# cxzheng/sprsolve

Measured on AMD Instinct MI355X. Metric: BiCGStab iterations/s (f64, 50M-row 7-point 3-D Poisson) + CSR SpMV GB/s vs HBM roofline, higher is better.
Workload: dtype f64

## Files before the change

### sprsolve_amd/csrc/capi.hip

```cpp
#include <sys/mman.h>

#include <cstdlib>
#include <memory>
#include <new>
#include <string>

#include "krylov.hpp"

using namespace sprs;

static_assert(sizeof(sprs_c64) == sizeof(cplx), "Complex<f64> layout");
static_assert(sizeof(sprs_c32) == sizeof(cplxf), "Complex<f32> layout");

#define SPRS_GUARD_BEGIN try {
#define SPRS_GUARD_END                         \
    }                                          \
    catch (const std::bad_alloc &) {           \
        return SPRS_ERR_HIP;                   \
    }                                          \
    catch (...) {                              \
        return SPRS_ERR_HIP;                   \
    }

extern "C" {
// ... 53 lines not shown
    (void)hipSetDevice(c->device);
    (void)hipStreamSynchronize(c->stream);
    if (c->d_part) (void)hipFree(c->d_part);
    if (c->d_scal) (void)hipFree(c->d_scal);
    if (c->h_scal) (void)hipHostFree(c->h_scal);
    if (c->own_stream && c->stream) (void)hipStreamDestroy(c->stream);
    delete c;
    return SPRS_OK;
}

int sprs_ctx_sync(sprs_ctx *c) {
    if (!c) return SPRS_INVALID_ARGUMENT;
    SPRS_HIP_TRY(c, hipStreamSynchronize(c->stream));
    return SPRS_OK;
}

const char *sprs_last_error(const sprs_ctx *c) { return c ? c->err : "null context"; }

int sprs_ctx_set(sprs_ctx *c, const char *key, int64_t value) {
    if (!c || !key) return SPRS_INVALID_ARGUMENT;
    std::string k(key);
    if (k == "grid") { if (value < 8 || value > MAX_GRID) return SPRS_INVALID_ARGUMENT; c->grid = (int)(value & ~7); }
    else if (k == "spmv_grid") { if (value > MAX_GRID / 2 || (value >= 0 && value < 8)) return SPRS_INVALID_ARGUMENT; c->spmv_grid = value < 0 ? -1 : (int)(value & ~7); }
    else if (k == "xcd_chunk") c->xcd_chunk = value < 0 ? -1 : (value ? 1 : 0);
    else if (k == "spmv_dict") { if (value < -1 || value > 2) return SPRS_INVALID_ARGUMENT; c->spmv_dict = (int)value; }
    else if (k == "spmv_wide") c->spmv_wide = value < 0 ? -1 : (value ? 1 : 0);
    else if (k == "spmv_uniform") c->spmv_uniform = value < 0 ? -1 : (value ? 1 : 0);
    else if (k == "spmv_period") c->spmv_period = value < 0 ? -1 : (value ? 1 : 0);
    else if (k == "spmv_triple") c->spmv_triple = value < 0 ? -1 : (value ? 1 : 0);
    else if (k == "spmv_seam") c->spmv_seam = value < 0 ? -1 : (value ? 1 : 0);
    else if (k == "spmv_tile") c->spmv_tile = value < 0 ? -1 : (value ? 1 : 0);
    else if (k == "spmv_chain") c->spmv_chain = value < 0 ? -1 : (value ? 1 : 0);
    else if (k == "spmv_fuse") c->spmv_fuse = value < 0 ? -1 : (value ? 1 : 0);
    else if (k == "bicg_k5") { if (value > 2) return SPRS_INVALID_ARGUMENT; c->bicg_k5 = value < 0 ? -1 : (int)value; }
    else if (k == "p2p_allreduce") c->p2p_allreduce = value < 0 ? -1 : (value ? 1 : 0);
    else if (k == "p2p_timeout_ms") c->p2p_timeout_ms = value < 1 ? 1 : value;
    else if (k == "ew_chunk") c->ew_chunk = value < 0 ? -1 : (value ? 1 : 0);
    else if (k == "stream_nt") c->stream_nt = value < 0 ? -1 : (value ? 1 : 0);
    else if (k == "spmv_eqrows") c->spmv_eqrows = value < 0 ? -1 : (value ? 1 : 0);
    else if (k == "spmv_wideload") c->spmv_wideload = value < 0 ? -1 : (value ? 1 : 0);
    else if (k == "halo_overlap") c->halo_overlap = value ? 1 : 0;
    else if (k == "gs_graph") c->gs_graph = value ? 1 : 0;
    else if (k == "poll") { if (value < 1) return SPRS_INVALID_ARGUMENT; c->poll = (int)value; }
    else return SPRS_INVALID_ARGUMENT;
    return SPRS_OK;
}
int64_t sprs_ctx_get(const sprs_ctx *c, const char *key) {
    if (!c || !key) return -1;
    std::string k(key);
    if (k == "grid") return c->grid;
    if (k == "xcd_chunk") return c->xcd_chunk;
    if (k == "spmv_grid") return c->spmv_grid;
    if (k == "spmv_dict") return c->spmv_dict;
    if (k == "spmv_wide") return c->spmv_wide;
    if (k == "spmv_uniform") return c->spmv_uniform;
    if (k == "spmv_period") return c->spmv_period;
    if (k == "spmv_triple") return c->spmv_triple;
    if (k == "spmv_seam") return c->spmv_seam;
    if (k == "spmv_tile") return c->spmv_tile;
    if (k == "spmv_chain") return c->spmv_chain;
    if (k == "spmv_fuse") return c->spmv_fuse;
    if (k == "bicg_k5") return c->bicg_k5;
    if (k == "p2p_allreduce") return c->p2p_allreduce;
    if (k == "p2p_timeout_ms") return c->p2p_timeout_ms;
    if (k == "ew_chunk") return c->ew_chunk;
    if (k == "stream_nt") return c->stream_nt;
    if (k == "spmv_eqrows") return c->spmv_eqrows;
    if (k == "spmv_wideload") return c->spmv_wideload;
    if (k == "halo_overlap") return c->halo_overlap;
    if (k == "gs_graph") return c->gs_graph;
    if (k == "poll") return c->poll;
    if (k == "num_cu") return c->num_cu;
    if (k == "device") return c->device;
    return -1;
}

int sprs_malloc(sprs_ctx *c, size_t bytes, void **dev_out) {
    if (!c || !dev_out) return SPRS_INVALID_ARGUMENT;
    SPRS_HIP_TRY(c, hipSetDevice(c->device));
    SPRS_HIP_TRY(c, hipMalloc(dev_out, bytes ? bytes : 16));
    return SPRS_OK;
}
int sprs_free(sprs_ctx *c, void *dev) {
    if (!c) return SPRS_INVALID_ARGUMENT;
    if (!dev) return SPRS_OK;
    SPRS_HIP_TRY(c, hipStreamSynchronize(c->stream));
    SPRS_HIP_TRY(c, hipFree(dev));
    return SPRS_OK;
}
int sprs_memcpy_h2d(sprs_ctx *c, void *d, const void *h, size_t bytes) {
    if (!c) return SPRS_INVALID_ARGUMENT;
    SPRS_HIP_TRY(c, hipMemcpyAsync(d, h, bytes, hipMemcpyHostToDevice, c->stream));
    SPRS_HIP_TRY(c, hipStreamSynchronize(c->stream));
    return SPRS_OK;
// ... 979 lines not shown
```

### sprsolve_amd/csrc/internal.hpp

```cpp
#pragma once
#include <hip/hip_runtime.h>
#include <hip/hip_ext.h>
#include <algorithm>
#include <cmath>
#include <cstdint>
#include <cstdio>
#include <cstring>
#include <cstdlib>
#include <ctime>
#include <mutex>
#include <type_traits>
#include <vector>

#include "../../include/sprsolve_hip.h"
#include "scalar.hpp"

namespace sprs {

constexpr int BLOCK = 256;
constexpr uint32_t UNI2 = 0x40000000u;
constexpr uint32_t SEAM2 = 0x20000000u;
constexpr int BICG_K5_DEFAULT = 1;
constexpr int MAX_GRID = 4096;

enum : int { ST_RUNNING = 0, ST_CONVERGED = 1, ST_RESTART = 2, ST_BREAKDOWN = 3, ST_INVALID_PC = 4,
             ST_COMM_TIMEOUT = 5 };

constexpr int MB_SLOTS = 4, MB_RANKS = 8, MB_GRAN = 8;
constexpr size_t MB_ENTRY = MB_GRAN * 8;
constexpr size_t MB_BYTES = (size_t)MB_SLOTS * 2 * MB_RANKS * MB_ENTRY;
inline size_t mb_offset(int slot, int parity) { return ((size_t)slot * 2 + (size_t)parity) * MB_RANKS * MB_ENTRY; }
struct P2pBox {
    unsigned long long peer[MB_RANKS];
    int world, rank;
};

struct Fin {
    unsigned int *counter = nullptr;
    const void *base0 = nullptr, *base1 = nullptr;
    void *out0 = nullptr, *out1 = nullptr;
    int P = 0;
    const P2pBox *box = nullptr;
    unsigned int tag = 0;
    unsigned int mb_off = 0;
};

}

struct sprs_ctx {
    int device = 0;
    hipStream_t stream = nullptr;
    bool own_stream = false;
    int num_cu = 256;
    int grid = 512;
    int spmv_grid = -1;
    int xcd_chunk = -1;
    int spmv_dict = -1;
    int spmv_wide = -1;
    int spmv_wideload = -1;
    int spmv_eqrows = -1;
    int spmv_period = -1;
    int spmv_triple = -1;
    int spmv_seam = -1;
    int spmv_tile = -1;
    int spmv_chain = -1;
    int spmv_fuse = -1;
    int bicg_k5 = -1;
    int ew_chunk = -1;
    int stream_nt = -1;
    int spmv_uniform = -1;
    int halo_overlap = 1;
    int gs_graph = 0;
    int p2p_allreduce = -1;
    int p2p_timeout_ms = 20000;
    int poll = 16;
    double *d_part = nullptr;
    double *d_scal = nullptr;
    double *h_scal = nullptr;
    mutable char err[512] = {0};
    hipEvent_t prof_start = nullptr, prof_stop = nullptr;
    mutable std::recursive_mutex mu;
};
struct CtxLock {
    std::unique_lock<std::recursive_mutex> lk;
    explicit CtxLock(const sprs_ctx *c) { if (c) lk = std::unique_lock<std::recursive_mutex>(c->mu); }
};

#define SPRS_HIP_TRY(ctx, expr)                                                                     \
    do {                                                                                            \
        hipError_t e__ = (expr);                                                                    \
        if (e__ != hipSuccess) {                                                                    \
            snprintf((ctx)->err, sizeof((ctx)->err), "%s:%d: %s -> %s", __FILE__, __LINE__, #expr,  \
                     hipGetErrorString(e__));                                                       \
            return SPRS_ERR_HIP;                                                                    \
        }                                                                                           \
    } while (0)

#define SPRS_LAUNCH_SPMV(c, kernel, grid, ...)                                                                            \
    do {                                                                                                                 \
// ... 15 lines not shown
        int s__ = (expr);                    \
        if (s__ != SPRS_OK) return s__;      \
    } while (0)

struct sprs_comm {
    sprs_ctx *ctx = nullptr;
    void *nccl = nullptr;
    int world = 1, rank = 0;
    bool p2p = false;
    void *mbox = nullptr;
    void *peer_map[8] = {nullptr};
    sprs::P2pBox *d_box = nullptr;
    unsigned int seq[4] = {0, 0, 0, 0};
};

struct sprs_tile_plan {
    int32_t *list = nullptr;
    int32_t *xstart = nullptr;
    int32_t *left = nullptr;
    int n_tile = 0, n_left = 0;
    int ul = 0, fl = 0, fh = 0;
    int w = 0;
    int32_t off[8] = {0, 0, 0, 0, 0, 0, 0, 0};
    double val[8] = {0, 0, 0, 0, 0, 0, 0, 0};
    std::vector<int32_t> h_list, h_xstart;
};

struct sprs_chain_plan {
    int32_t *tiles = nullptr;
    int32_t *segs = nullptr;
    int32_t *xstart = nullptr;
    int32_t *left = nullptr;
    int n_tile = 0, n_seg = 0, n_chain = 0, n_left = 0;
    int ul = 0, tri = 0;
    int32_t off[8] = {0, 0, 0, 0, 0, 0, 0, 0};
    double val[8] = {0, 0, 0, 0, 0, 0, 0, 0};
};

struct sprs_dist_info {
    sprs_comm *comm = nullptr;
    int64_t n_local = 0, n_ext = 0;
    std::vector<int> peer;
    std::vector<int64_t> send_off, recv_off;
    int32_t *send_idx = nullptr;
    void *send_buf = nullptr;
    int64_t ag_slice = 0;
    void *ag_buf = nullptr;
    int32_t *order_int = nullptr, *order_bnd = nullptr;
    int32_t n_int = 0, n_bnd = 0;
    int32_t *order_int_w = nullptr, *order_bnd_w = nullptr;
    sprs_tile_plan tile_int;
    bool tile_int_off = false;
    int32_t n_int_w = 0, n_bnd_w = 0;
    hipStream_t comm_stream = nullptr;
    hipEvent_t ev_pack = nullptr, ev_halo = nullptr;
};

struct sprs_dict {
    uint8_t *idx_code = nullptr;
    uint8_t *pair_code = nullptr;
    int32_t *off_tab = nullptr;
    int32_t *pair_off = nullptr;
    void *pair_val = nullptr;
    void *rowval = nullptr;
    int n_off = 0, n_val = 0, n_pair = 0;
    void *wide_desc = nullptr;
// ... 271 lines not shown
```

### sprsolve_amd/csrc/spmv_chain.hip

```cpp
#include "spmv_dict_dev.hpp"
#include "bicg_fuse.hpp"

namespace sprs {
namespace {

constexpr int CH_ROWS = CH_B * 2 * WAVE;
constexpr int CH_W = TILE_W;
constexpr int CH_WL = CH_ROWS + 2 * CH_W;

struct NoPro { __device__ __forceinline__ bool prologue() { return true; } };
template <int FUSE, class PRO, int DOT, bool UX, int UL, bool TRI, bool YST = true, int UPD = 0>
__global__ __launch_bounds__(BLOCK) void spmv_chain_kernel(const int4 *__restrict__ tiles, const int2 *__restrict__ segs, const int32_t *__restrict__ xstart,
                                                           const BlkDesc *__restrict__ desc, const TilePat pat,
                                                           int n_left, const int32_t *__restrict__ left_order,
                                                           const int32_t *__restrict__ row_ptr, const uint8_t *__restrict__ code,
                                                           const int32_t *__restrict__ off_tab, const double *__restrict__ val_tab,
                                                           const double *__restrict__ x, double *__restrict__ y, const double *__restrict__ u,
                                                           double *__restrict__ part0, double *__restrict__ part1,
                                                           const int *__restrict__ status, int nrows, int ncols, const Fin fin,
                                                           PRO pro, const double *__restrict__ in1, const double *__restrict__ in2,
                                                           double *__restrict__ own) {
    using T = double;
    constexpr int NV = FUSE == 0 ? 1 : FUSE;
    static_assert(FUSE == 0 || (FUSE == 2 && DOT == 2 && UX && UPD == 0) || (FUSE == 3 && DOT == 1 && !UX) ||
                  (FUSE == 2 && DOT == 0 && !UX && !YST && UPD != 0), "fused flavours: K3 into K4, K1 into K2, K5 on the chains");
    static_assert((YST || FUSE == 2) && (UPD == 0 || FUSE == 2), "only BiCGStab's K4 / K5 drop the y store");
    constexpr int W = CH_W, WL = CH_WL;
    constexpr int NW = WL / 2 / BLOCK;
    constexpr int NQ = CH_B / NWAVE;
    constexpr int NN = UL - 2;
    constexpr int TC = NN / 2;
    static_assert(WL % (2 * BLOCK) == 0 && CH_B % NWAVE == 0 && NN >= 1 && UL <= 8 && (!TRI || (NN & 1)), "chain shape");
    static_assert(sizeof(T) * WL >= sizeof(uint32_t) * NWAVE * CW2, "the left walk's code slices live in the first window");
    __shared__ __attribute__((aligned(16))) T win[3][WL];
    __shared__ PairEnt<T> s_pair[TAB];
    __shared__ T red[NWAVE];
    const int run_state = status != nullptr ? *status : (int)ST_RUNNING;
    const int tid = threadIdx.x, lane = tid & (WAVE - 1);
    const int wv = __builtin_amdgcn_readfirstlane(tid >> 6);
    stage_pair(s_pair, tid, off_tab[tid] * 8, val_tab[tid]);
    __syncthreads();
    if (run_state != ST_RUNNING) { fin_idle(fin, DOT == 2); return; }
    [[maybe_unused]] T c0 = 0.0, c1 = 0.0;
    [[maybe_unused]] T nw = 0.0;
    if constexpr (FUSE != 0) {
        if (!pro.prologue()) return;
        if constexpr (FUSE == 2) c0 = pro.na; else { c0 = pro.a; c1 = pro.beta; }
        if constexpr (UPD != 0) nw = pro.nw;
    }
    T d0 = 0.0, d1 = 0.0;

    const int Pf = pat.off[UL - 1];
    const int xhi = (ncols - 2) & ~1;
    const int xcd = blockIdx.x & 7;
    const int sstep = gridDim.x >> 3;
    const int send = xstart[xcd + 1];
    constexpr int PF = (FUSE == 3 || UPD != 0) ? 1 : 2;
    struct WinRegs { u4v a[NW]; u4v b[NV >= 2 ? NW : 1]; u4v c[NV == 3 ? NW : 1]; };
    WinRegs R0;
    [[maybe_unused]] WinRegs R1;
    auto issue = [&](int tw, WinRegs &R) {
#pragma unroll
        for (int i = 0; i < NW; ++i) {
            int g = tw - W + 2 * (tid + i * BLOCK);
            g = g < 0 ? 0 : (g > xhi ? xhi : g);
            R.a[i] = *reinterpret_cast<const u4v *>(x + g);
            if constexpr (NV >= 2) R.b[i] = *reinterpret_cast<const u4v *>(in1 + g);
            if constexpr (NV == 3) R.c[i] = *reinterpret_cast<const u4v *>(in2 + g);
        }
    };
    auto stage = [&](int slot, const WinRegs &R) {
#pragma unroll
        for (int i = 0; i < NW; ++i) {
            if constexpr (FUSE == 0) {
                *reinterpret_cast<u4v *>(&win[slot][2 * (tid + i * BLOCK)]) = R.a[i];
            } else {
                D2 a, b, cc{0.0, 0.0};
                __builtin_memcpy(&a, &R.a[i], 16); __builtin_memcpy(&b, &R.b[i], 16);
                if constexpr (NV == 3) __builtin_memcpy(&cc, &R.c[i], 16);
                const D2 o = FUSE == 2 ? D2{comb_k3(a.lo, b.lo, c0), comb_k3(a.hi, b.hi, c0)}
                                       : D2{comb_k1(a.lo, b.lo, cc.lo, c0, c1), comb_k1(a.hi, b.hi, cc.hi, c0, c1)};
                *reinterpret_cast<D2 *>(&win[slot][2 * (tid + i * BLOCK)]) = o;
            }
        }
    };
    for (int s = xstart[xcd] + (blockIdx.x >> 3); s < send; s += sstep) {
        const int2 sg = segs[s];
        const int t0 = __builtin_amdgcn_readfirstlane(sg.x), L = __builtin_amdgcn_readfirstlane(sg.y);
        int4 ent = tiles[t0];
        uint32_t rbw[NQ]; int nnw[NQ];
#pragma unroll
        for (int q = 0; q < NQ; ++q) { const BlkDesc d = desc[__builtin_amdgcn_readfirstlane(ent.x) + q * NWAVE + wv]; rbw[q] = (uint32_t)d.rb; nnw[q] = d.nn; }
        __syncthreads();
        int ts_prev = __builtin_amdgcn_readfirstlane(ent.y) - Pf;
        int sp = 0, sc = 1, sn = 2;
        issue(ts_prev, R0); stage(sp, R0);
        issue(__builtin_amdgcn_readfirstlane(ent.y), R0); stage(sc, R0);
        issue(__builtin_amdgcn_readfirstlane(ent.z), R0);
        if constexpr (PF == 2) { if (L > 1) issue(tiles[t0 + 1].z, R1); }
        auto body = [&](int k, WinRegs &RS) {
            const int ts = __builtin_amdgcn_readfirstlane(ent.y), ts_next = __builtin_amdgcn_readfirstlane(ent.z);
            uint32_t rbc[NQ]; int nnc[NQ];
#pragma unroll
            for (int q = 0; q < NQ; ++q) { rbc[q] = rbw[q]; nnc[q] = nnw[q]; }
            stage(sn, RS);
            __syncthreads();
            if (k + PF < L) issue(tiles[t0 + k + PF].z, RS);
            if (k + 1 < L) {
                ent = tiles[t0 + k + 1];
                const int b1 = __builtin_amdgcn_readfirstlane(ent.x);
#pragma unroll
                for (int q = 0; q < NQ; ++q) { const BlkDesc d = desc[b1 + q * NWAVE + wv]; rbw[q] = (uint32_t)d.rb; nnw[q] = d.nn; }
            }
            const int dlo = ts - Pf - ts_prev, dhi = ts + Pf - ts_next;
            const T *wp = &win[sp][W + dlo], *wc = &win[sc][W], *wn = &win[sn][W + dhi];
            D2 uu[NQ];
            if (DOT != 0 && !UX) {
#pragma unroll
                for (int q = 0; q < NQ; ++q) {
                    const u4v w4 = __builtin_nontemporal_load(reinterpret_cast<const u4v *>(u + (ts + ((q * NWAVE + wv) << 7) + 2 * lane)));
                    __builtin_memcpy(&uu[q], &w4, 16);
                }
            }
            struct UpdRegs { u4v x, p, q, t; };
            [[maybe_unused]] UpdRegs ur[2];
            [[maybe_unused]] auto upd_load = [&](int q, UpdRegs &U) {
                if constexpr (UPD != 0) {
                    const int g = ts + ((q * NWAVE + wv) << 7) + 2 * lane;
                    U.x = __builtin_nontemporal_load(reinterpret_cast<const u4v *>(pro.x + g));
                    U.p = __builtin_nontemporal_load(reinterpret_cast<const u4v *>(pro.y + g));
// ... 45 lines not shown
                }
                row_pair_out<DOT, YST>(y + (ts + ((q * NWAVE + wv) << 7) + 2 * lane), acc0, acc1, u0, u1, d0, d1);
                if constexpr (UPD != 0) {
                    D2 xx, pp, qq, rr;
                    __builtin_memcpy(&xx, &ur[q & 1].x, 16); __builtin_memcpy(&pp, &ur[q & 1].p, 16); __builtin_memcpy(&qq, &ur[q & 1].q, 16);
                    bicg_k5_row(xx.lo, pp.lo, mine.lo, acc0, qq.lo, c0, nw, rr.lo, d0, d1);
                    bicg_k5_row(xx.hi, pp.hi, mine.hi, acc1, qq.hi, c0, nw, rr.hi, d0, d1);
                    const int g = ts + ((q * NWAVE + wv) << 7) + 2 * lane;
                    u4v xo, ro;
                    __builtin_memcpy(&xo, &xx, 16); __builtin_memcpy(&ro, &rr, 16);
                    __builtin_nontemporal_store(xo, reinterpret_cast<u4v *>(pro.x + g));
                    __builtin_nontemporal_store(ro, reinterpret_cast<u4v *>(own + g));
                }
                if constexpr (FUSE == 3) {
                    u4v ov;
                    __builtin_memcpy(&ov, &mine, 16);
                    __builtin_nontemporal_store(ov, reinterpret_cast<u4v *>(own + (ts + ((q * NWAVE + wv) << 7) + 2 * lane)));
                }
            }
            __syncthreads();
            ts_prev = ts;
            const int o = sp; sp = sc; sc = sn; sn = o;
        };
        if constexpr (PF == 2) {
            for (int k = 0; k < L; k += 2) { body(k, R0); if (k + 1 < L) body(k + 1, R1); }
        } else {
            for (int k = 0; k < L; ++k) body(k, R0);
        }
    }
    if (n_left > 0) {
        __syncthreads();
        uint32_t (*s_c)[CW2] = reinterpret_cast<uint32_t (*)[CW2]>(&win[0][0]);
        for (int i = lane; i < CW2; i += WAVE) s_c[wv][i] = 0;
        if constexpr (FUSE == 0)
            pair2_walk<DOT, true>(n_left, 0, desc, left_order, row_ptr, code, XPlain{reinterpret_cast<const char *>(x)}, y, u, nrows, ncols, s_pair, s_c, d0, d1);
        else if constexpr (UPD != 0)
            pair2_walk<0, true, XFused<2>, false, BicgUpd<UPD>>(n_left, 0, desc, left_order, row_ptr, code,
                                                                XFused<2>{reinterpret_cast<const char *>(x), reinterpret_cast<const char *>(in1), nullptr, c0, c1},
                                                                nullptr, nullptr, nrows, ncols, s_pair, s_c, d0, d1, nullptr,
                                                                BicgUpd<UPD>{pro.x, pro.y, pro.r0, pro.t, own, c0, nw});
        else if constexpr (!YST)
            pair2_walk<DOT, true, XFused<NV>, false>(n_left, 0, desc, left_order, row_ptr, code,
                                                     XFused<NV>{reinterpret_cast<const char *>(x), reinterpret_cast<const char *>(in1), reinterpret_cast<const char *>(in2), c0, c1},
                                                     nullptr, UX ? nullptr : u, nrows, ncols, s_pair, s_c, d0, d1, own);
        else
            pair2_walk<DOT, true, XFused<NV>>(n_left, 0, desc, left_order, row_ptr, code,
                                              XFused<NV>{reinterpret_cast<const char *>(x), reinterpret_cast<const char *>(in1), reinterpret_cast<const char *>(in2), c0, c1},
                                              y, UX ? nullptr : u, nrows, ncols, s_pair, s_c, d0, d1, own);
    }
    spmv_dot_epilogue<DOT>(d0, d1, red, part0, part1, fin);
    if constexpr (UPD != 0) {
        pro.accN = d0; pro.accR = d1;
        pro.epilogue();
    }
}

}

int chain_rows() { return CH_ROWS; }

template <class Kern, class PRO>
int launch_chain(const sprs_csr *A, const SpmvRoute &rt, Kern kern, const double *x, double *y, const double *u, double *part0, double *part1,
                 const int *status, const Fin &fin, const PRO &pro, const double *in1, const double *in2, double *own) {
    sprs_ctx *c = A->ctx;
    const sprs_dict *D = A->dict;
    const sprs_chain_plan &CP = *rt.chain;
    const TilePat tp = tile_pat(CP);
#define SPRS_CSHAPE(U, TR)                                                                                                                 \
    if (CP.ul == U && (CP.tri != 0) == TR)                                                                                                 \
        SPRS_LAUNCH_SPMV(c, kern(std::integral_constant<int, U>{}, std::bool_constant<TR>{}), rt.grid, reinterpret_cast<const int4 *>(CP.tiles), \
                         reinterpret_cast<const int2 *>(CP.segs), CP.xstart, rt.desc, tp, CP.n_left, CP.left, A->row_ptr, D->pair_code, D->pair_off, \
                         reinterpret_cast<const double *>(D->pair_val), x, y, u, part0, part1, status, (int)A->nrows, (int)A->ncols, fin, pro, in1, in2, own);
    SPRS_CHAIN_SHAPES(SPRS_CSHAPE)
#undef SPRS_CSHAPE
    SPRS_HIP_TRY(c, hipGetLastError());
    return SPRS_OK;
}

int launch_chain_pair(const sprs_csr *A, const SpmvRoute &r, const double *x, double *y, int dot_mode, const double *u,
                      double *part0, double *part1, const int *status, const Fin &fin) {
    int rc = SPRS_OK;
    with_dot(dot_mode, u == x, [&](auto dm, auto ux) {
        constexpr int DM = decltype(dm)::value;
        constexpr bool UXV = DM != 0 && decltype(ux)::value;
        rc = launch_chain(A, r, [](auto ul, auto tri) { return &spmv_chain_kernel<0, NoPro, DM, UXV, decltype(ul)::value, decltype(tri)::value>; },
                          x, y, u, part0, part1, status, fin, NoPro{}, nullptr, nullptr, nullptr);
    });
    return rc;
}

int launch_chain_k4f(const sprs_csr *A, const SpmvRoute &rt, const BicgK3<double, double, false> &pro, const double *r, const double *v, double *s_out,
                     double *t, double *partTT, double *partTR, const int *status, bool store_t) {
    typedef BicgK3<double, double, false> K3;
    auto go = [&](auto yst) {
        return launch_chain(A, rt, [](auto ul, auto tri) { return &spmv_chain_kernel<2, K3, 2, true, decltype(ul)::value, decltype(tri)::value, decltype(yst)::value>; },
                            r, t, nullptr, partTT, partTR, status, Fin{}, pro, v, nullptr, s_out);
    };
    return store_t ? go(std::true_type{}) : go(std::false_type{});
}

int launch_chain_k5(const sprs_csr *A, const SpmvRoute &rt, const BicgK5<double, false, true> &pro, double *r_out, bool recompute) {
    typedef BicgK5<double, false, true> K5;
    auto go = [&](auto upd) {
        return launch_chain(A, rt, [](auto ul, auto tri) { return &spmv_chain_kernel<2, K5, 0, false, decltype(ul)::value, decltype(tri)::value, false, decltype(upd)::value>; },
// ... 14 lines not shown
```

### sprsolve_amd/csrc/spmv_dict.hip

```cpp
#include <algorithm>
#include <cstring>
#include <map>

#include "spmv_dict_dev.hpp"
#include "minres_fuse.hpp"

namespace sprs {

namespace {

constexpr int HSLOTS = 1024;
constexpr uint32_t EMPTY32 = 0x80000000u;
constexpr uint64_t EMPTY64 = 0xFFFFFFFFFFFFFFFFull;

__device__ __forceinline__ uint32_t hash32(uint32_t k) { k ^= k >> 16; k *= 0x7feb352du; k ^= k >> 15; k *= 0x846ca68bu; k ^= k >> 16; return k; }
__device__ __forceinline__ uint32_t hash64(uint64_t k) { k ^= k >> 33; k *= 0xff51afd7ed558ccdull; k ^= k >> 33; return (uint32_t)k; }

__device__ __forceinline__ uint64_t key_of(double v) { return (uint64_t)__double_as_longlong(v); }
__device__ __forceinline__ uint64_t key_of(float v) { return (uint64_t)__float_as_uint(v); }

__device__ __forceinline__ int probe32(uint32_t *tab, int *count, uint32_t key, bool insert) {
    uint32_t h = hash32(key) & (HSLOTS - 1);
    for (int t = 0; t < HSLOTS; ++t, h = (h + 1) & (HSLOTS - 1)) {
        uint32_t cur = __hip_atomic_load(tab + h, __ATOMIC_RELAXED, __HIP_MEMORY_SCOPE_AGENT);
// ... 418 lines not shown
            }
            const uint32_t mB8 = mB == full ? 0xffu : (uint32_t)mB;
            const uint32_t rbw = UNI2 | SEAM2 | mB8 | ((uint32_t)(cA < 0 ? 0 : cA) << 8) | ((uint32_t)(cB < 0 ? 0 : cB) << 16) |
                                 (cA >= 0 ? 1u << 24 : 0u) | (cB >= 0 ? 1u << 25 : 0u);
            desc[b] = BlkDesc{d.ra, (int32_t)rbw, pA, Lmax | (centre << 8) | (k << 16) | (mA << 23)};
        }
    }
}

template <int DOT, bool YNT>
__global__ __launch_bounds__(BLOCK) void spmv_pair2_kernel(int n_wide, int xcd_chunk, const BlkDesc *__restrict__ desc,
                                                           const int32_t *__restrict__ order,
                                                           const int32_t *__restrict__ row_ptr,
                                                           const uint8_t *__restrict__ code,
                                                           const int32_t *__restrict__ off_tab,
                                                           const double *__restrict__ val_tab, const double *__restrict__ x,
                                                           double *__restrict__ y, const double *__restrict__ u,
                                                           double *__restrict__ part0, double *__restrict__ part1,
                                                           const int *__restrict__ status, int nrows, int ncols, const Fin fin) {
    using T = double;
    __shared__ PairEnt<T> s_pair[TAB];
    __shared__ __attribute__((aligned(16))) uint32_t s_c[NWAVE][CW2];
    __shared__ T red[NWAVE];
    const int run_state = status != nullptr ? *status : (int)ST_RUNNING;

    const int tid = threadIdx.x, lane = tid & (WAVE - 1);
    const int wv = __builtin_amdgcn_readfirstlane(tid >> 6);
    stage_pair(s_pair, tid, off_tab[tid] * 8, val_tab[tid]);
    for (int i = lane; i < CW2; i += WAVE) s_c[wv][i] = 0;
    __syncthreads();
    if (run_state != ST_RUNNING) { fin_idle(fin, DOT == 2); return; }

    T d0 = 0.0, d1 = 0.0;
    pair2_walk<DOT, YNT>(n_wide, xcd_chunk, desc, order, row_ptr, code, XPlain{reinterpret_cast<const char *>(x)}, y, u, nrows, ncols, s_pair, s_c, d0, d1);
    spmv_dot_epilogue<DOT>(d0, d1, red, part0, part1, fin);
}

__global__ __launch_bounds__(BLOCK) void tile_mark_kernel(int n_cand, const BlkDesc *__restrict__ desc, const uint8_t *__restrict__ code,
                                                          unsigned long long *__restrict__ pat_out, int *__restrict__ len_out) {
    const int t = blockIdx.x * BLOCK + threadIdx.x;
    if (t >= n_cand) return;
    unsigned long long pat0 = 0;
    int L0 = 0, ra0 = 0;
    bool ok = true;
    for (int i = 0; i < TILE_B && ok; ++i) {
        const BlkDesc d = desc[t * TILE_B + i];
        const uint32_t rb = (uint32_t)d.rb;
        ok = (rb & UNI2) != 0;
        if (!ok) break;
        const bool seam = (rb & SEAM2) != 0;
        const int L = d.nn & 0xff;
        const int nr = seam ? 2 * WAVE : (int)(rb & ~UNI2) - d.ra;
        unsigned long long pat = 0;
        for (int j = 0; j < L && j < 8; ++j) pat |= (unsigned long long)code[d.pa + j] << (8 * j);
        if (i == 0) { pat0 = pat; L0 = L; ra0 = d.ra; }
        ok = nr == 2 * WAVE && L == L0 && L >= 1 && L <= 8 && pat == pat0 && d.ra == ra0 + i * 2 * WAVE;
    }
    pat_out[t] = ok ? pat0 : 0ull;
    len_out[t] = ok ? L0 : 0;
}

__global__ __launch_bounds__(BLOCK) void tile_flag_kernel(int n_wide, const BlkDesc *__restrict__ desc, const uint8_t *__restrict__ code,
                                                          unsigned long long pat, int L, uint8_t *__restrict__ flag) {
    const int j = blockIdx.x * BLOCK + threadIdx.x;
    if (j >= n_wide) return;
    const BlkDesc d = desc[j];
    const uint32_t rb = (uint32_t)d.rb;
// ... 135 lines not shown
                const auto &idv = ids[(size_t)(ci - c_lo)];
                segs.push_back((int32_t)(tiles.size() / 4)); segs.push_back(sv[k].second);
                for (int p2 = sv[k].first; p2 < sv[k].first + sv[k].second; ++p2) {
                    const int ti = idv[(size_t)p2];
                    const int b0 = tb[(size_t)ti];
                    const int32_t ra = wd[(size_t)b0].ra;
                    const int32_t ra_next = next[(size_t)ti] >= 0 ? wd[(size_t)tb[(size_t)next[(size_t)ti]]].ra : (int32_t)(ra + Pf);
                    tiles.push_back(b0); tiles.push_back(ra); tiles.push_back(ra_next); tiles.push_back(0);
                    for (int qb = 0; qb < CH_B; ++qb) in_chain[(size_t)(b0 + qb)] = 1;
                    covered += CH_B;
                }
                ++n_seg;
            }
    }
    xstart[8] = n_seg;
    const int n_tile = (int)(tiles.size() / 4);
    const bool fills = n_seg * 2 >= G && covered * 2 >= flagged && n_tile >= 6 * n_seg;
    if (n_tile == 0 || (c->spmv_chain < 0 && !fills)) return SPRS_OK;
    std::vector<int32_t> left;
    make_left(in_chain, left);
    auto drop = [&]() { for (void *q : {(void *)CP.tiles, (void *)CP.segs, (void *)CP.xstart, (void *)CP.left}) if (q) (void)hipFree(q); CP = sprs_chain_plan(); };
#define CH_TRY(expr) do { hipError_t e__ = (expr); if (e__ != hipSuccess) { snprintf(c->err, sizeof(c->err), "%s:%d: %s -> %s", __FILE__, __LINE__, #expr, hipGetErrorString(e__)); drop(); return SPRS_ERR_HIP; } } while (0)
    CH_TRY(hipMalloc((void **)&CP.tiles, sizeof(int32_t) * tiles.size()));
    CH_TRY(hipMalloc((void **)&CP.segs, sizeof(int32_t) * segs.size()));
    CH_TRY(hipMalloc((void **)&CP.xstart, sizeof(int32_t) * 9));
    CH_TRY(hipMalloc((void **)&CP.left, sizeof(int32_t) * std::max<size_t>(left.size(), 1)));
    CH_TRY(hipMemcpyAsync(CP.tiles, tiles.data(), sizeof(int32_t) * tiles.size(), hipMemcpyHostToDevice, c->stream));
    CH_TRY(hipMemcpyAsync(CP.segs, segs.data(), sizeof(int32_t) * segs.size(), hipMemcpyHostToDevice, c->stream));
    CH_TRY(hipMemcpyAsync(CP.xstart, xstart.data(), sizeof(int32_t) * 9, hipMemcpyHostToDevice, c->stream));
    if (!left.empty()) CH_TRY(hipMemcpyAsync(CP.left, left.data(), sizeof(int32_t) * left.size(), hipMemcpyHostToDevice, c->stream));
    CH_TRY(hipStreamSynchronize(c->stream));
#undef CH_TRY
    CP.n_tile = n_tile; CP.n_seg = n_seg; CP.n_chain = nch; CP.n_left = (int)left.size();
    CP.ul = UL; CP.tri = tri ? 1 : 0;
    for (int t = 0; t < 8; ++t) { CP.off[t] = t < UL ? off[t] : 0; CP.val[t] = t < UL ? val[t] : 0.0; }
    return SPRS_OK;
}

template <class MakeLeft>
static int build_tile_plan(sprs_csr *A, sprs_tile_plan &TP, const BlkDesc *desc_dev, const uint8_t *code_dev, const std::vector<BlkDescHost2> &wd,
                           const int32_t *off_tab, const double *val_tab, bool wide_window_ok, MakeLeft &&make_left, sprs_chain_plan *CP = nullptr) {
    sprs_ctx *c = A->ctx;
    const int nw = (int)wd.size();
    const int n_cand = nw / TILE_B;
    if (!(tile_wanted(c, (size_t)A->nrows * sizeof(double)) && c->spmv_uniform != 0 && c->spmv_wide != 0 && n_cand >= 16 && A->ncols >= TILE_ROWS + 2 * TILE_W)) return SPRS_OK;
    unsigned long long *pat_d = nullptr; int *len_d = nullptr; uint8_t *flag_d = nullptr;
    auto drop = [&]() { for (void *q : {(void *)pat_d, (void *)len_d, (void *)flag_d}) if (q) (void)hipFree(q); pat_d = nullptr; len_d = nullptr; flag_d = nullptr; };
#define TILE_TRY(expr) do { hipError_t e__ = (expr); if (e__ != hipSuccess) { snprintf(c->err, sizeof(c->err), "%s:%d: %s -> %s", __FILE__, __LINE__, #expr, hipGetErrorString(e__)); drop(); return SPRS_ERR_HIP; } } while (0)
    TILE_TRY(hipMalloc((void **)&pat_d, sizeof(unsigned long long) * (size_t)n_cand));
    TILE_TRY(hipMalloc((void **)&len_d, sizeof(int) * (size_t)n_cand));
    hipLaunchKernelGGL(tile_mark_kernel, dim3((n_cand + BLOCK - 1) / BLOCK), dim3(BLOCK), 0, c->stream, n_cand, desc_dev, code_dev, pat_d, len_d);
    TILE_TRY(hipGetLastError());
    std::vector<unsigned long long> h_pat((size_t)n_cand);
    std::vector<int> h_len((size_t)n_cand);
    TILE_TRY(hipMemcpyAsync(h_pat.data(), pat_d, sizeof(unsigned long long) * (size_t)n_cand, hipMemcpyDeviceToHost, c->stream));
    TILE_TRY(hipMemcpyAsync(h_len.data(), len_d, sizeof(int) * (size_t)n_cand, hipMemcpyDeviceToHost, c->stream));
    TILE_TRY(hipStreamSynchronize(c->stream));
    std::map<std::pair<unsigned long long, int>, int> hist;
    for (int t = 0; t < n_cand; ++t) if (h_len[(size_t)t] > 0) ++hist[{h_pat[(size_t)t], h_len[(size_t)t]}];
    std::pair<unsigned long long, int> canon{0ull, 0};
    int best = 0;
    for (const auto &kv : hist) if (kv.second > best) { best = kv.second; canon = kv.first; }
    const int UL = canon.second;
    int FL = 0, FH = 0, WIN = 0;
    bool shape_ok = false;
    int64_t far_band = 0;
// ... 494 lines not shown
```

### sprsolve_amd/csrc/spmv_dict_dev.hpp

```cpp
#pragma once
#include "device.hpp"

namespace sprs {

struct alignas(16) V2d { double a, b; };

namespace {

constexpr int TAB = 256;

constexpr int CPAD = 16;

template <class T> struct alignas(sizeof(T) >= 8 ? 16 : 8) PairEnt { int32_t off8; T val; };
template <class T>
__device__ __forceinline__ void stage_pair(PairEnt<T> *s_pair, int i, int32_t off8, T val) {
    s_pair[i].off8 = off8;
    s_pair[i].val = val;
}

template <class T, bool PAIR, int ITEMS>
struct BlkLoads {
    int ra, rb, pa, nn;
    int ulen;
    int s;
// ... 363 lines not shown
        for (int t = 0; t < 8; ++t) {
            if (UL == 0 ? t >= ulen : t >= UL) break;
            acc0 = acc0 + pl[t] * av[t];
            acc1 = acc1 + ph[t] * av[t];
        }
    } else {
        seam_fold_masked<UL>(pl, ph, av, ulen, seam1, seam2, s_pair, lane, acc0, acc1);
    }
}
template <class XS, class AfterLoads>
__device__ __forceinline__ void full_uniform_dispatch(const PairEnt<double> *s_pair, uint64_t pat, int ulen, int sc, bool seam, int seam1, int seam2, const XS &xs,
                                                      uint32_t r8, uint32_t ra8, int lane, AfterLoads &&after_loads,
                                                      double &acc0, double &acc1) {
    if (ulen == 7 && sc == 3) full_uniform_block<7, 3>(s_pair, pat, ulen, seam, seam1, seam2, xs, r8, ra8, lane, after_loads, acc0, acc1);
    else if (ulen == 5 && sc == 2) full_uniform_block<5, 2>(s_pair, pat, ulen, seam, seam1, seam2, xs, r8, ra8, lane, after_loads, acc0, acc1);
    else if (ulen == 3 && sc == 1) full_uniform_block<3, 1>(s_pair, pat, ulen, seam, seam1, seam2, xs, r8, ra8, lane, after_loads, acc0, acc1);
    else full_uniform_block<0, 0>(s_pair, pat, ulen, seam, seam1, seam2, xs, r8, ra8, lane, after_loads, acc0, acc1);
}


struct Blk2Loads {
    int ra, rb, pa, nn;
    bool uni; int ulen;
    int tri;
    bool is_seam; int seam1, seam2;
    int a, b;
    double u0, u1;
    double o0, o1;
    D2 kx, kp, kq, kt;
    u4v wc;
    int di;
};

template <int DOT, bool YNT, class XS = XPlain, bool YST = true, class UP = NoUpd>
__device__ __forceinline__ void pair2_walk(int n_wide, int xcd_chunk, const BlkDesc *__restrict__ desc,
                                           const int32_t *__restrict__ order, const int32_t *__restrict__ row_ptr,
                                           const uint8_t *__restrict__ code, const XS xs,
                                           double *__restrict__ y, const double *__restrict__ u, int nrows, int ncols,
                                           const PairEnt<double> *s_pair, uint32_t (*s_c)[CW2], double &d0, double &d1,
                                           double *__restrict__ own = nullptr, const UP up = UP{}) {
    using T = double;
    static_assert(UP::MODE == 0 || (XS::FUSED && DOT == 0 && !YST), "the update needs s from the walk and owns both running sums");
    const int tid = threadIdx.x, lane = tid & (WAVE - 1);
    const int wv = __builtin_amdgcn_readfirstlane(tid >> 6);
    const uint8_t *cb = reinterpret_cast<const uint8_t *>(s_c[wv]);
    const uint32_t xlast_pair = (uint32_t)(ncols - 2) * 8u;
    const bool u_is_x = XS::FUSED && u == nullptr;

    int b, bstep, bend;
    if (xcd_chunk) {
        const int chunk = (n_wide + 7) >> 3;
        const int xcd = blockIdx.x & 7;
        b = xcd * chunk + (blockIdx.x >> 3) * NWAVE + wv;
        bstep = (gridDim.x >> 3) * NWAVE;
        bend = min(n_wide, (xcd + 1) * chunk);
    } else {
        b = blockIdx.x * NWAVE + wv; bstep = gridDim.x * NWAVE; bend = n_wide;
    }
    if (b >= bend) b = bend;

    typedef const int32_t __attribute__((address_space(1))) *gi32_p;
    uintptr_t order_a = reinterpret_cast<uintptr_t>(order);
    asm volatile("" : "+v"(order_a));
    const gi32_p order_v = reinterpret_cast<gi32_p>(order_a);
    auto load_desc = [&](int bi) -> BlkDesc { return desc[bi]; };
    auto block_index = [&](int bi) -> int { return order ? order_v[bi] : bi; };
    auto uniform = [&](const BlkDesc &d) -> BlkDesc {
        return BlkDesc{__builtin_amdgcn_readfirstlane(d.ra), __builtin_amdgcn_readfirstlane(d.rb),
                       __builtin_amdgcn_readfirstlane(d.pa), __builtin_amdgcn_readfirstlane(d.nn)};
    };
    auto issue = [&](const BlkDesc &d, Blk2Loads &L) {
        L.uni = ((uint32_t)d.rb & UNI2) != 0;
        L.is_seam = L.uni && ((uint32_t)d.rb & SEAM2) != 0;
        L.ra = d.ra; L.rb = L.is_seam ? d.ra + 2 * WAVE : (int)((uint32_t)d.rb & ~UNI2); L.pa = d.pa;
        L.ulen = L.uni ? (d.nn & 0xff) : 0;
        L.tri = L.uni ? ((d.nn >> 8) & 0xff) : 0;
        L.seam1 = L.is_seam ? (d.nn >> 16) : 0;
        L.seam2 = L.is_seam ? (int)((uint32_t)d.rb & 0x3ffffffu) : 0;
        L.nn = L.uni ? L.ulen * (L.rb - L.ra) : d.nn;
        const int r0 = L.ra + 2 * lane;
        L.a = 0; L.b = 0;
        if (!L.uni) {
            const int i0 = min(r0, L.rb - 1);
            const int2 ab = *reinterpret_cast<const int2 *>(reinterpret_cast<const char *>(row_ptr) + (uint32_t)i0 * 4u);
            L.a = ab.x; L.b = ab.y;
        }
        if (DOT != 0 && !u_is_x) {
            const int p0 = min(r0, nrows - 2);
            const D2 uu = *reinterpret_cast<const D2 *>(reinterpret_cast<const char *>(u) + (uint32_t)p0 * 8u);
            L.u0 = r0 == p0 ? uu.lo : uu.hi;
            L.u1 = uu.hi;
// ... 290 lines not shown
```

### sprsolve_amd/csrc/spmv_tile.hip

```cpp
#include "spmv_dict_dev.hpp"

namespace sprs {
namespace {

template <int DOT, bool UX, int UL, int FL, int FH, int W>
__global__ __launch_bounds__(BLOCK) void spmv_tile_kernel(const int2 *__restrict__ tile_list, const int32_t *__restrict__ xstart,
                                                          const BlkDesc *__restrict__ desc, const TilePat pat,
                                                          int n_left, const int32_t *__restrict__ left_order,
                                                          const int32_t *__restrict__ row_ptr, const uint8_t *__restrict__ code,
                                                          const int32_t *__restrict__ off_tab, const double *__restrict__ val_tab,
                                                          const double *__restrict__ x, double *__restrict__ y, const double *__restrict__ u,
                                                          double *__restrict__ part0, double *__restrict__ part1,
                                                          const int *__restrict__ status, int nrows, int ncols, const Fin fin) {
    using T = double;
    constexpr int TR = TILE_ROWS;
    constexpr int NW = (TR + 2 * W) / 2 / BLOCK;
    constexpr int NQ = TILE_B / NWAVE;
    constexpr int NN = UL - FL - FH;
    static_assert((TR + 2 * W) % (2 * BLOCK) == 0 && TILE_B % NWAVE == 0 && NN >= 1 && UL <= 8, "tile shape");
    __shared__ __attribute__((aligned(16))) T win[TR + 2 * W];
    __shared__ PairEnt<T> s_pair[TAB];
    __shared__ __attribute__((aligned(16))) uint32_t s_c[NWAVE][CW2];
    __shared__ T red[NWAVE];
    const int run_state = status != nullptr ? *status : (int)ST_RUNNING;
// ... 10 lines not shown
    tile_seam_words(desc, __builtin_amdgcn_readfirstlane(cur.ent.x), wv, rbw, nnw);
    for (; cur.s < cur.send; cur.s += cur.sstep) {
        const int ts = tile_cursor_take(cur, tile_list);
        uint32_t rbc[NQ]; int nnc[NQ];
#pragma unroll
        for (int q = 0; q < NQ; ++q) { rbc[q] = rbw[q]; nnc[q] = nnw[q]; }
        u4v wreg[NW];
        window_load(x + (ts - W), tid, wreg);
        D2 far[NQ][FL + FH > 0 ? FL + FH : 1];
        D2 uu[NQ];
#pragma unroll
        for (int q = 0; q < NQ; ++q) tile_far_loads<DOT, UX, UL, FL, FH>(x, u, pat, ts + ((q * NWAVE + wv) << 7) + 2 * lane, far[q], uu[q]);
        if (cur.s + cur.sstep < cur.send) tile_seam_words(desc, __builtin_amdgcn_readfirstlane(cur.ent.x), wv, rbw, nnw);
        window_stage(win, tid, wreg);
        T npl[NN], nph[NN];
        tile_read_near(win, W + (wv << 7) + 2 * lane, pat.off + FL, npl, nph);
#pragma unroll
        for (int q = 0; q < NQ; ++q) {
            const uint32_t rbq = (uint32_t)__builtin_amdgcn_readfirstlane((int)rbc[q]);
            const int li = W + ((q * NWAVE + wv) << 7) + 2 * lane;
            T pl[UL], ph[UL];
            tile_slots<UL, FL, FH>(far[q], npl, nph, pl, ph);
            T ux0 = 0.0, ux1 = 0.0;
            if (DOT != 0 && UX) { ux0 = win[li]; ux1 = win[li + 1]; }
            if (q + 1 < NQ) tile_read_near(win, W + (((q + 1) * NWAVE + wv) << 7) + 2 * lane, pat.off + FL, npl, nph);
            T acc0 = 0.0, acc1 = 0.0;
            pair_fold<UL>(pl, ph, pat.val, rbq, nnc[q], s_pair, lane, acc0, acc1);
            row_pair_out<DOT>(y + (ts + ((q * NWAVE + wv) << 7) + 2 * lane), acc0, acc1, (DOT != 0 && !UX) ? uu[q].lo : ux0,
                              (DOT != 0 && !UX) ? uu[q].hi : ux1, d0, d1);
        }
    }
    if (n_left > 0) {
        __syncthreads();
        pair2_walk<DOT, true>(n_left, 0, desc, left_order, row_ptr, code, XPlain{reinterpret_cast<const char *>(x)}, y, u, nrows, ncols, s_pair, s_c, d0, d1);
    }
    spmv_dot_epilogue<DOT>(d0, d1, red, part0, part1, fin);
}

}

int launch_tile_pair(const sprs_csr *A, const SpmvRoute &r, const double *x, double *y, int dot_mode, const double *u,
                     double *part0, double *part1, const int *status, const Fin &fin) {
    sprs_ctx *c = A->ctx;
    const sprs_dict *D = A->dict;
    const sprs_tile_plan &TP = *r.tile;
    const double *pvd = reinterpret_cast<const double *>(D->pair_val);
    const TilePat tp = tile_pat(TP);
    with_dot(dot_mode, u == x, [&](auto dm, auto ux) {
        constexpr int DM = decltype(dm)::value;
        constexpr bool UXV = DM != 0 && decltype(ux)::value;
#define SPRS_TSHAPE(U, L, H)                                                                                                              \
    if (TP.ul == U && TP.fl == L && TP.fh == H)                                                                                           \
        SPRS_LAUNCH_SPMV(c, (spmv_tile_kernel<DM, UXV, U, L, H, SPRS_TW>), r.grid, reinterpret_cast<const int2 *>(TP.list), TP.xstart, r.desc, tp, \
                         TP.n_left, TP.left, A->row_ptr, D->pair_code, D->pair_off, pvd, x, y, u, part0, part1, status, (int)A->nrows, (int)A->ncols, fin);
#define SPRS_TW TILE_W
        if (TP.w == TILE_W) { SPRS_TILE_SHAPES(SPRS_TSHAPE) }
#undef SPRS_TW
#define SPRS_TW TILE_W_WIDE
        if (TP.w == TILE_W_WIDE) { SPRS_TILE_SHAPES_WIDE(SPRS_TSHAPE) }
#undef SPRS_TW
#undef SPRS_TSHAPE
    });
    SPRS_HIP_TRY(c, hipGetLastError());
    return SPRS_OK;
}

}
// ... 1 lines not shown
```

Before: 883.4.

## Prefetch first chain segment before staging and assign leftover rows to idle blocks

The chain SpMV kernel now issues the first segment's tile and window loads before staging the pair table and running the fused prologue, so that memory latency overlaps the setup work. It also adds an optional two-pass split of the leftover (non-chained) rows: blocks with no chain segment first take a share sized from the longest segment, then every block walks the remainder. pair2_walk is refactored to take a WalkRange. The leftover split is off by default (CHAIN_LEFT_DEFAULT=0), so only the prefetch reordering is active, and it raises register pressure.

```diff
diff --git a/sprsolve_amd/csrc/capi.hip b/sprsolve_amd/csrc/capi.hip
--- a/sprsolve_amd/csrc/capi.hip
+++ b/sprsolve_amd/csrc/capi.hip
@@ -109,6 +109,7 @@
     else if (k == "spmv_tile") c->spmv_tile = value < 0 ? -1 : (value ? 1 : 0);
     else if (k == "spmv_chain") c->spmv_chain = value < 0 ? -1 : (value ? 1 : 0);
     else if (k == "spmv_fuse") c->spmv_fuse = value < 0 ? -1 : (value ? 1 : 0);
+    else if (k == "chain_left") { if (value > (1 << 20)) return SPRS_INVALID_ARGUMENT; c->chain_left = value < 0 ? -1 : (int)value; }
     else if (k == "bicg_k5") { if (value > 2) return SPRS_INVALID_ARGUMENT; c->bicg_k5 = value < 0 ? -1 : (int)value; }
     else if (k == "p2p_allreduce") c->p2p_allreduce = value < 0 ? -1 : (value ? 1 : 0);
     else if (k == "p2p_timeout_ms") c->p2p_timeout_ms = value < 1 ? 1 : value;
@@ -137,6 +138,7 @@
     if (k == "spmv_tile") return c->spmv_tile;
     if (k == "spmv_chain") return c->spmv_chain;
     if (k == "spmv_fuse") return c->spmv_fuse;
+    if (k == "chain_left") return c->chain_left;
     if (k == "bicg_k5") return c->bicg_k5;
     if (k == "p2p_allreduce") return c->p2p_allreduce;
     if (k == "p2p_timeout_ms") return c->p2p_timeout_ms;
diff --git a/sprsolve_amd/csrc/internal.hpp b/sprsolve_amd/csrc/internal.hpp
--- a/sprsolve_amd/csrc/internal.hpp
+++ b/sprsolve_amd/csrc/internal.hpp
@@ -21,6 +21,8 @@
 constexpr uint32_t UNI2 = 0x40000000u;
 constexpr uint32_t SEAM2 = 0x20000000u;
 constexpr int BICG_K5_DEFAULT = 1;
+constexpr int CHAIN_LEFT_DEFAULT = 0;
+constexpr double CHAIN_LEFT_KAPPA = 0.71;
 constexpr int MAX_GRID = 4096;
 
 enum : int { ST_RUNNING = 0, ST_CONVERGED = 1, ST_RESTART = 2, ST_BREAKDOWN = 3, ST_INVALID_PC = 4,
@@ -65,6 +67,7 @@
     int spmv_tile = -1;
     int spmv_chain = -1;
     int spmv_fuse = -1;
+    int chain_left = -1;
     int bicg_k5 = -1;
     int ew_chunk = -1;
     int stream_nt = -1;
@@ -146,6 +149,8 @@
     int32_t *xstart = nullptr;
     int32_t *left = nullptr;
     int n_tile = 0, n_seg = 0, n_chain = 0, n_left = 0;
+    int max_seg = 0;
+    std::vector<int32_t> h_xstart;
     int ul = 0, tri = 0;
     int32_t off[8] = {0, 0, 0, 0, 0, 0, 0, 0};
     double val[8] = {0, 0, 0, 0, 0, 0, 0, 0};
diff --git a/sprsolve_amd/csrc/spmv_chain.hip b/sprsolve_amd/csrc/spmv_chain.hip
--- a/sprsolve_amd/csrc/spmv_chain.hip
+++ b/sprsolve_amd/csrc/spmv_chain.hip
@@ -8,11 +8,12 @@
 constexpr int CH_W = TILE_W;
 constexpr int CH_WL = CH_ROWS + 2 * CH_W;
 
+struct ChainLeft { int n_idle_left, n_idle; uint16_t base[8]; };
 struct NoPro { __device__ __forceinline__ bool prologue() { return true; } };
 template <int FUSE, class PRO, int DOT, bool UX, int UL, bool TRI, bool YST = true, int UPD = 0>
 __global__ __launch_bounds__(BLOCK) void spmv_chain_kernel(const int4 *__restrict__ tiles, const int2 *__restrict__ segs, const int32_t *__restrict__ xstart,
                                                            const BlkDesc *__restrict__ desc, const TilePat pat,
-                                                           int n_left, const int32_t *__restrict__ left_order,
+                                                           int n_left, const ChainLeft cl, const int32_t *__restrict__ left_order,
                                                            const int32_t *__restrict__ row_ptr, const uint8_t *__restrict__ code,
                                                            const int32_t *__restrict__ off_tab, const double *__restrict__ val_tab,
                                                            const double *__restrict__ x, double *__restrict__ y, const double *__restrict__ u,
@@ -38,23 +39,13 @@
     const int run_state = status != nullptr ? *status : (int)ST_RUNNING;
     const int tid = threadIdx.x, lane = tid & (WAVE - 1);
     const int wv = __builtin_amdgcn_readfirstlane(tid >> 6);
-    stage_pair(s_pair, tid, off_tab[tid] * 8, val_tab[tid]);
-    __syncthreads();
-    if (run_state != ST_RUNNING) { fin_idle(fin, DOT == 2); return; }
     [[maybe_unused]] T c0 = 0.0, c1 = 0.0;
     [[maybe_unused]] T nw = 0.0;
-    if constexpr (FUSE != 0) {
-        if (!pro.prologue()) return;
-        if constexpr (FUSE == 2) c0 = pro.na; else { c0 = pro.a; c1 = pro.beta; }
-        if constexpr (UPD != 0) nw = pro.nw;
-    }
-    T d0 = 0.0, d1 = 0.0;
-
     const int Pf = pat.off[UL - 1];
     const int xhi = (ncols - 2) & ~1;
     const int xcd = blockIdx.x & 7;
     const int sstep = gridDim.x >> 3;
-    const int send = xstart[xcd + 1];
+    const int sbeg = xstart[xcd], send = xstart[xcd + 1];
     constexpr int PF = (FUSE == 3 || UPD != 0) ? 1 : 2;
     struct WinRegs { u4v a[NW]; u4v b[NV >= 2 ? NW : 1]; u4v c[NV == 3 ? NW : 1]; };
     WinRegs R0;
@@ -84,18 +75,43 @@
             }
         }
     };
-    for (int s = xstart[xcd] + (blockIdx.x >> 3); s < send; s += sstep) {
-        const int2 sg = segs[s];
+    int s = sbeg + (blockIdx.x >> 3);
+    bool primed = s < send;
+    int2 sg{0, 0};
+    int4 ent{0, 0, 0, 0};
+    if (primed) {
+        sg = segs[s];
+        ent = tiles[__builtin_amdgcn_readfirstlane(sg.x)];
+        issue(__builtin_amdgcn_readfirstlane(ent.y) - Pf, R0);
+        if constexpr (PF == 2) issue(__builtin_amdgcn_readfirstlane(ent.y), R1);
+    }
+    stage_pair(s_pair, tid, off_tab[tid] * 8, val_tab[tid]);
+    __syncthreads();
+    if (run_state != ST_RUNNING) { fin_idle(fin, DOT == 2); return; }
+    if constexpr (FUSE != 0) {
+        if (!pro.prologue()) return;
+        if constexpr (FUSE == 2) c0 = pro.na; else { c0 = pro.a; c1 = pro.beta; }
+        if constexpr (UPD != 0) nw = pro.nw;
+    }
+    T d0 = 0.0, d1 = 0.0;
+
+    for (; s < send; s += sstep) {
+        if (!primed) { sg = segs[s]; ent = tiles[__builtin_amdgcn_readfirstlane(sg.x)]; }
         const int t0 = __builtin_amdgcn_readfirstlane(sg.x), L = __builtin_amdgcn_readfirstlane(sg.y);
-        int4 ent = tiles[t0];
         uint32_t rbw[NQ]; int nnw[NQ];
 #pragma unroll
         for (int q = 0; q < NQ; ++q) { const BlkDesc d = desc[__builtin_amdgcn_readfirstlane(ent.x) + q * NWAVE + wv]; rbw[q] = (uint32_t)d.rb; nnw[q] = d.nn; }
         __syncthreads();
         int ts_prev = __builtin_amdgcn_readfirstlane(ent.y) - Pf;
         int sp = 0, sc = 1, sn = 2;
-        issue(ts_prev, R0); stage(sp, R0);
-        issue(__builtin_amdgcn_readfirstlane(ent.y), R0); stage(sc, R0);
+        if (!primed) {
+            issue(ts_prev, R0);
+            if constexpr (PF == 2) issue(__builtin_amdgcn_readfirstlane(ent.y), R1);
+        }
+        primed = false;
+        stage(sp, R0);
+        if constexpr (PF == 2) { stage(sc, R1); }
+        else { issue(__builtin_amdgcn_readfirstlane(ent.y), R0); stage(sc, R0); }
         issue(__builtin_amdgcn_readfirstlane(ent.z), R0);
         if constexpr (PF == 2) { if (L > 1) issue(tiles[t0 + 1].z, R1); }
         auto body = [&](int k, WinRegs &RS) {
@@ -207,21 +223,28 @@
         __syncthreads();
         uint32_t (*s_c)[CW2] = reinterpret_cast<uint32_t (*)[CW2]>(&win[0][0]);
         for (int i = lane; i < CW2; i += WAVE) s_c[wv][i] = 0;
-        if constexpr (FUSE == 0)
-            pair2_walk<DOT, true>(n_left, 0, desc, left_order, row_ptr, code, XPlain{reinterpret_cast<const char *>(x)}, y, u, nrows, ncols, s_pair, s_c, d0, d1);
-        else if constexpr (UPD != 0)
-            pair2_walk<0, true, XFused<2>, false, BicgUpd<UPD>>(n_left, 0, desc, left_order, row_ptr, code,
-                                                                XFused<2>{reinterpret_cast<const char *>(x), reinterpret_cast<const char *>(in1), nullptr, c0, c1},
-                                                                nullptr, nullptr, nrows, ncols, s_pair, s_c, d0, d1, nullptr,
-                                                                BicgUpd<UPD>{pro.x, pro.y, pro.r0, pro.t, own, c0, nw});
-        else if constexpr (!YST)
-            pair2_walk<DOT, true, XFused<NV>, false>(n_left, 0, desc, left_order, row_ptr, code,
-                                                     XFused<NV>{reinterpret_cast<const char *>(x), reinterpret_cast<const char *>(in1), reinterpret_cast<const char *>(in2), c0, c1},
-                                                     nullptr, UX ? nullptr : u, nrows, ncols, s_pair, s_c, d0, d1, own);
-        else
-            pair2_walk<DOT, true, XFused<NV>>(n_left, 0, desc, left_order, row_ptr, code,
-                                              XFused<NV>{reinterpret_cast<const char *>(x), reinterpret_cast<const char *>(in1), reinterpret_cast<const char *>(in2), c0, c1},
-                                              y, UX ? nullptr : u, nrows, ncols, s_pair, s_c, d0, d1, own);
+        const int widx = (int)(blockIdx.x >> 3) - (send - sbeg);
+        const WalkRange idle_rg{((int)cl.base[xcd] + widx) * NWAVE + wv, cl.n_idle * NWAVE, cl.n_idle_left};
+        const WalkRange grid_rg{cl.n_idle_left + (int)blockIdx.x * NWAVE + wv, (int)gridDim.x * NWAVE, n_left};
+#pragma clang loop unroll(disable)
+        for (int pass = (cl.n_idle_left > 0 && widx >= 0) ? 0 : 1; pass < 2; ++pass) {
+            const WalkRange rg = pass == 0 ? idle_rg : grid_rg;
+            if constexpr (FUSE == 0)
+                pair2_walk<DOT, true>(rg, desc, left_order, row_ptr, code, XPlain{reinterpret_cast<const char *>(x)}, y, u, nrows, ncols, s_pair, s_c, d0, d1);
+            else if constexpr (UPD != 0)
+                pair2_walk<0, true, XFused<2>, false, BicgUpd<UPD>>(rg, desc, left_order, row_ptr, code,
+                                                                    XFused<2>{reinterpret_cast<const char *>(x), reinterpret_cast<const char *>(in1), nullptr, c0, c1},
+                                                                    nullptr, nullptr, nrows, ncols, s_pair, s_c, d0, d1, nullptr,
+                                                                    BicgUpd<UPD>{pro.x, pro.y, pro.r0, pro.t, own, c0, nw});
+            else if constexpr (!YST)
+                pair2_walk<DOT, true, XFused<NV>, false>(rg, desc, left_order, row_ptr, code,
+                                                         XFused<NV>{reinterpret_cast<const char *>(x), reinterpret_cast<const char *>(in1), reinterpret_cast<const char *>(in2), c0, c1},
+                                                         nullptr, UX ? nullptr : u, nrows, ncols, s_pair, s_c, d0, d1, own);
+            else
+                pair2_walk<DOT, true, XFused<NV>>(rg, desc, left_order, row_ptr, code,
+                                                  XFused<NV>{reinterpret_cast<const char *>(x), reinterpret_cast<const char *>(in1), reinterpret_cast<const char *>(in2), c0, c1},
+                                                  y, UX ? nullptr : u, nrows, ncols, s_pair, s_c, d0, d1, own);
+        }
     }
     spmv_dot_epilogue<DOT>(d0, d1, red, part0, part1, fin);
     if constexpr (UPD != 0) {
@@ -241,10 +264,22 @@
     const sprs_dict *D = A->dict;
     const sprs_chain_plan &CP = *rt.chain;
     const TilePat tp = tile_pat(CP);
+    ChainLeft cl{};
+    const int mode = c->chain_left < 0 ? CHAIN_LEFT_DEFAULT : c->chain_left;
+    if (mode != 0 && CP.n_left > 0) {
+        int idle = 0;
+        for (int xq = 0; xq < 8; ++xq) {
+            cl.base[xq] = (uint16_t)idle;
+            idle += std::max(0, (rt.grid >> 3) - (CP.h_xstart[(size_t)xq + 1] - CP.h_xstart[(size_t)xq]));
+        }
+        const int64_t m = mode == 1 ? (int64_t)std::ceil(CHAIN_LEFT_KAPPA * CP.max_seg) : mode;
+        cl.n_idle = idle;
+        cl.n_idle_left = (int)std::min<int64_t>(CP.n_left, (int64_t)NWAVE * idle * m);
+    }
 #define SPRS_CSHAPE(U, TR)                                                                                                                 \
     if (CP.ul == U && (CP.tri != 0) == TR)                                                                                                 \
         SPRS_LAUNCH_SPMV(c, kern(std::integral_constant<int, U>{}, std::bool_constant<TR>{}), rt.grid, reinterpret_cast<const int4 *>(CP.tiles), \
-                         reinterpret_cast<const int2 *>(CP.segs), CP.xstart, rt.desc, tp, CP.n_left, CP.left, A->row_ptr, D->pair_code, D->pair_off, \
+                         reinterpret_cast<const int2 *>(CP.segs), CP.xstart, rt.desc, tp, CP.n_left, cl, CP.left, A->row_ptr, D->pair_code, D->pair_off, \
                          reinterpret_cast<const double *>(D->pair_val), x, y, u, part0, part1, status, (int)A->nrows, (int)A->ncols, fin, pro, in1, in2, own);
     SPRS_CHAIN_SHAPES(SPRS_CSHAPE)
 #undef SPRS_CSHAPE
diff --git a/sprsolve_amd/csrc/spmv_dict.hip b/sprsolve_amd/csrc/spmv_dict.hip
--- a/sprsolve_amd/csrc/spmv_dict.hip
+++ b/sprsolve_amd/csrc/spmv_dict.hip
@@ -474,7 +474,7 @@
     if (run_state != ST_RUNNING) { fin_idle(fin, DOT == 2); return; }
 
     T d0 = 0.0, d1 = 0.0;
-    pair2_walk<DOT, YNT>(n_wide, xcd_chunk, desc, order, row_ptr, code, XPlain{reinterpret_cast<const char *>(x)}, y, u, nrows, ncols, s_pair, s_c, d0, d1);
+    pair2_walk<DOT, YNT>(walk_range(n_wide, xcd_chunk), desc, order, row_ptr, code, XPlain{reinterpret_cast<const char *>(x)}, y, u, nrows, ncols, s_pair, s_c, d0, d1);
     spmv_dot_epilogue<DOT>(d0, d1, red, part0, part1, fin);
 }
 
@@ -676,6 +676,8 @@
     CH_TRY(hipStreamSynchronize(c->stream));
 #undef CH_TRY
     CP.n_tile = n_tile; CP.n_seg = n_seg; CP.n_chain = nch; CP.n_left = (int)left.size();
+    CP.h_xstart = xstart; CP.max_seg = 0;
+    for (size_t k = 1; k < segs.size(); k += 2) CP.max_seg = std::max(CP.max_seg, (int)segs[k]);
     CP.ul = UL; CP.tri = tri ? 1 : 0;
     for (int t = 0; t < 8; ++t) { CP.off[t] = t < UL ? off[t] : 0; CP.val[t] = t < UL ? val[t] : 0.0; }
     return SPRS_OK;
diff --git a/sprsolve_amd/csrc/spmv_dict_dev.hpp b/sprsolve_amd/csrc/spmv_dict_dev.hpp
--- a/sprsolve_amd/csrc/spmv_dict_dev.hpp
+++ b/sprsolve_amd/csrc/spmv_dict_dev.hpp
@@ -419,8 +419,25 @@
     int di;
 };
 
+struct WalkRange { int first, step, end; };
+__device__ __forceinline__ WalkRange walk_range(int n, int xcd_chunk) {
+    const int tid = threadIdx.x;
+    const int wv = __builtin_amdgcn_readfirstlane(tid >> 6);
+    WalkRange r;
+    if (xcd_chunk) {
+        const int chunk = (n + 7) >> 3;
+        const int xcd = blockIdx.x & 7;
+        r.first = xcd * chunk + (blockIdx.x >> 3) * NWAVE + wv;
+        r.step = (gridDim.x >> 3) * NWAVE;
+        r.end = min(n, (xcd + 1) * chunk);
+    } else {
+        r.first = blockIdx.x * NWAVE + wv; r.step = gridDim.x * NWAVE; r.end = n;
+    }
+    return r;
+}
+
 template <int DOT, bool YNT, class XS = XPlain, bool YST = true, class UP = NoUpd>
-__device__ __forceinline__ void pair2_walk(int n_wide, int xcd_chunk, const BlkDesc *__restrict__ desc,
+__device__ __forceinline__ void pair2_walk(const WalkRange rg, const BlkDesc *__restrict__ desc,
                                            const int32_t *__restrict__ order, const int32_t *__restrict__ row_ptr,
                                            const uint8_t *__restrict__ code, const XS xs,
                                            double *__restrict__ y, const double *__restrict__ u, int nrows, int ncols,
@@ -434,16 +451,8 @@
     const uint32_t xlast_pair = (uint32_t)(ncols - 2) * 8u;
     const bool u_is_x = XS::FUSED && u == nullptr;
 
-    int b, bstep, bend;
-    if (xcd_chunk) {
-        const int chunk = (n_wide + 7) >> 3;
-        const int xcd = blockIdx.x & 7;
-        b = xcd * chunk + (blockIdx.x >> 3) * NWAVE + wv;
-        bstep = (gridDim.x >> 3) * NWAVE;
-        bend = min(n_wide, (xcd + 1) * chunk);
-    } else {
-        b = blockIdx.x * NWAVE + wv; bstep = gridDim.x * NWAVE; bend = n_wide;
-    }
+    int b = rg.first;
+    const int bstep = rg.step, bend = rg.end;
     if (b >= bend) b = bend;
 
     typedef const int32_t __attribute__((address_space(1))) *gi32_p;
diff --git a/sprsolve_amd/csrc/spmv_tile.hip b/sprsolve_amd/csrc/spmv_tile.hip
--- a/sprsolve_amd/csrc/spmv_tile.hip
+++ b/sprsolve_amd/csrc/spmv_tile.hip
@@ -66,7 +66,7 @@
     }
     if (n_left > 0) {
         __syncthreads();
-        pair2_walk<DOT, true>(n_left, 0, desc, left_order, row_ptr, code, XPlain{reinterpret_cast<const char *>(x)}, y, u, nrows, ncols, s_pair, s_c, d0, d1);
+        pair2_walk<DOT, true>(walk_range(n_left, 0), desc, left_order, row_ptr, code, XPlain{reinterpret_cast<const char *>(x)}, y, u, nrows, ncols, s_pair, s_c, d0, d1);
     }
     spmv_dot_epilogue<DOT>(d0, d1, red, part0, part1, fin);
 }
```

After: 889.5, median of 6. About the same (+0.7%).
